# indrajeetadityaroy9/rabitq-ann-search

Measured on AMD Instinct MI355X. Metric: qps (search_batch_device, layer-0 hot path end to end) + fastscan_dist_per_s, higher is better.
Workload: dtype u32 popcount / f32; 1 GPU; SIFT1M-class synthetic (int-valued, clustered; SURVEY 8d C2): 1000000x128 f32 (D=128), 4-bit RaBitQ FastScan + exact-L2 rerank, R=32, k=10, 10000 queries per GPU resident in HBM; n_index=1000000, dim=128, bits=4, k=10, nq_per_gpu=10000, index_builder=cphnsw_mi355x (this repo), batch_sets=2, parallelism=query-sharded x1, index replicated

## Files before the change

include/cphnsw_mi355x.h:

```cpp
#ifndef CPHNSW_MI355X_H
#define CPHNSW_MI355X_H

#include <stddef.h>
#include <stdint.h>

#ifdef __cplusplus
extern "C" {
#endif

typedef struct cph_index cph_index;

typedef enum {
    CPH_OK = 0,
    CPH_INVALID_ARGUMENT = 1,
    CPH_RUNTIME_ERROR = 2,
    CPH_OUT_OF_MEMORY = 3,
    CPH_NOT_IMPLEMENTED = 4
} cph_status;

const char* cph_last_error(void);

int cph_version(void);

int cph_create(uint64_t dim, uint64_t bits, int device, cph_index** out);
// ... 229 lines not shown
int cph_debug_time_facets(cph_index* h, int on);
int cph_debug_last_facets_us(cph_index* h, double* us);
int cph_debug_facet_slab(cph_index* h, uint64_t counters);
int cph_host_facet_values(const int32_t* column, uint64_t n_entries, const uint64_t* lims, uint64_t n, uint64_t* U, int32_t* values);
int cph_host_facet_counts(const int32_t* column, uint64_t n_entries, const uint64_t* lims, uint64_t n, const uint32_t* words,
                          const uint32_t* removed, uint32_t m, uint64_t* counts_out);
int cph_host_facet_top(const int32_t* column, uint64_t n_entries, const uint64_t* lims, uint64_t n, const uint32_t* words,
                       const uint32_t* removed, uint32_t m, uint32_t K, int32_t* values_out, uint64_t* counts_out, uint32_t* found_out);
int cph_facet_hook(int device, const uint32_t* codes, uint64_t n_entries, const uint32_t* lims, uint64_t n, uint32_t U,
                   const uint32_t* words, uint32_t m, int path, uint64_t* counts_out, double* kernel_us);

int cph_search(cph_index* h, const float* query, uint64_t k, int64_t* ids, float* dist,
               uint64_t* m);

int cph_get_vectors(cph_index* h, uint64_t first, uint64_t count, float* out);

int cph_set_batch_sets(cph_index* h, uint32_t n_sets);

int cph_set_search_params(cph_index* h, uint32_t slots, uint64_t beam_capacity);

int cph_last_search_stats(cph_index* h, uint64_t out[12]);
int cph_last_query_expansions(cph_index* index, uint32_t* out, uint64_t n);
int cph_order_queries(cph_index* index, const float* keys, uint64_t n, uint32_t* order);

typedef struct cph_multi cph_multi;
int cph_multi_create(uint64_t dim, uint64_t bits, const int* devices, uint32_t n_dev, cph_multi** out);
int cph_multi_destroy(cph_multi* m);
int cph_multi_load(cph_multi* m, const char* path);
int cph_multi_load_native(cph_multi* m, const char* path);
int cph_multi_save(cph_multi* m, const char* path);
int cph_multi_save_native(cph_multi* m, const char* path);
int cph_multi_build(cph_multi* m, const float* vectors, uint64_t n);
int cph_multi_finalize(cph_multi* m);
int cph_multi_size(cph_multi* m, uint64_t* n);
int cph_multi_is_finalized(cph_multi* m, int* flag);
int cph_multi_search_batch(cph_multi* m, const float* queries, uint64_t n, uint64_t k, int64_t* ids, float* dist);
int cph_multi_search_batch_filtered(cph_multi* m, const float* queries, uint64_t n, uint64_t k,
                                    const cph_filter* const* f, int64_t* ids, float* dist);
int cph_multi_search_batch_exact(cph_multi* m, const float* queries, uint64_t n, uint64_t k,
                                 const cph_filter* const* f, int64_t* ids, float* dist);
int cph_multi_search_batch_filters(cph_multi* m, const float* queries, uint64_t n, uint64_t k, const cph_filter* const* filters,
                                   uint32_t n_filters, const int32_t* filter_of, int exact, int64_t* ids, float* dist);
typedef struct cph_multi_range cph_multi_range;
int cph_multi_range_search_begin(cph_multi* m, const float* queries, uint64_t n, const float* radius_host,
                                 const cph_filter* const* f, int exact, uint64_t max_results, cph_multi_range** out,
                                 uint64_t* total);
// ... 190 lines not shown
```

rabitq-ann-search_amd/cphnsw_mi355x/_lib.py:

```python
import ctypes as C
import importlib.util
import os
import sys

from . import build as _build

OK, INVALID_ARGUMENT, RUNTIME_ERROR, OUT_OF_MEMORY, NOT_IMPLEMENTED = range(5)
IDS_INTERNAL, IDS_INPUT = 0, 1
METRIC_L2, METRIC_COSINE = 0, 1
METRIC_IP = 2

SYMBOLS = {
    "cph_last_error": (C.c_char_p, []),
    "cph_version": (C.c_int, []),
    "cph_create": (C.c_int, [C.c_uint64, C.c_uint64, C.c_int, C.POINTER(C.c_void_p)]),
    "cph_destroy": (C.c_int, [C.c_void_p]),
    "cph_load": (C.c_int, [C.c_void_p, C.c_char_p]),
    "cph_save": (C.c_int, [C.c_void_p, C.c_char_p]),
    "cph_save_native": (C.c_int, [C.c_void_p, C.c_char_p]),
    "cph_load_native": (C.c_int, [C.c_void_p, C.c_char_p]),
    "cph_size": (C.c_int, [C.c_void_p, C.POINTER(C.c_uint64)]),
    "cph_dim": (C.c_int, [C.c_void_p, C.POINTER(C.c_uint64)]),
    "cph_is_finalized": (C.c_int, [C.c_void_p, C.POINTER(C.c_int)]),
    "cph_build": (C.c_int, [C.c_void_p, C.c_void_p, C.c_uint64]),
# ... 183 lines not shown
    "cph_facet_counts": (C.c_int, [C.c_void_p, C.c_int, C.c_uint32, C.c_void_p, C.c_uint32, C.c_void_p]),
    "cph_facet_top": (C.c_int, [C.c_void_p, C.c_int, C.c_uint32, C.c_void_p, C.c_uint32, C.c_uint32, C.c_void_p, C.c_void_p, C.c_void_p]),
    "cph_debug_time_facets": (C.c_int, [C.c_void_p, C.c_int]),
    "cph_debug_last_facets_us": (C.c_int, [C.c_void_p, C.POINTER(C.c_double)]),
    "cph_debug_facet_slab": (C.c_int, [C.c_void_p, C.c_uint64]),
    "cph_host_facet_values": (C.c_int, [C.c_void_p, C.c_uint64, C.c_void_p, C.c_uint64, C.POINTER(C.c_uint64), C.c_void_p]),
    "cph_host_facet_counts": (C.c_int, [C.c_void_p, C.c_uint64, C.c_void_p, C.c_uint64, C.c_void_p, C.c_void_p, C.c_uint32, C.c_void_p]),
    "cph_host_facet_top": (C.c_int, [C.c_void_p, C.c_uint64, C.c_void_p, C.c_uint64, C.c_void_p, C.c_void_p, C.c_uint32, C.c_uint32,
                                     C.c_void_p, C.c_void_p, C.c_void_p]),
    "cph_facet_hook": (C.c_int, [C.c_int, C.c_void_p, C.c_uint64, C.c_void_p, C.c_uint64, C.c_uint32, C.c_void_p, C.c_uint32, C.c_int,
                                 C.c_void_p, C.POINTER(C.c_double)]),
    "cph_multi_set_tags": (C.c_int, [C.c_void_p, C.c_uint32, C.c_void_p, C.c_void_p, C.c_uint64, C.c_int]),
    "cph_parts_set_tags": (C.c_int, [C.c_void_p, C.c_uint32, C.c_void_p, C.c_void_p, C.c_uint64]),
    "cph_parts_filters_from_tags": (C.c_int, [C.c_void_p, C.c_uint32, C.c_void_p, C.c_void_p, C.c_void_p, C.c_uint32, C.c_void_p]),
    "cph_synchronize": (C.c_int, [C.c_void_p]),
    "cph_set_batch_sets": (C.c_int, [C.c_void_p, C.c_uint32]),
    "cph_search": (C.c_int, [C.c_void_p, C.c_void_p, C.c_uint64, C.c_void_p, C.c_void_p,
                             C.POINTER(C.c_uint64)]),
    "cph_get_vectors": (C.c_int, [C.c_void_p, C.c_uint64, C.c_uint64, C.c_void_p]),
    "cph_set_search_params": (C.c_int, [C.c_void_p, C.c_uint32, C.c_uint64]),
    "cph_last_search_stats": (C.c_int, [C.c_void_p, C.POINTER(C.c_uint64)]),
    "cph_last_query_expansions": (C.c_int, [C.c_void_p, C.c_void_p, C.c_uint64]),
    "cph_order_queries": (C.c_int, [C.c_void_p, C.c_void_p, C.c_uint64, C.c_void_p]),
    "cph_multi_create": (C.c_int, [C.c_uint64, C.c_uint64, C.c_void_p, C.c_uint32, C.POINTER(C.c_void_p)]),
    "cph_multi_destroy": (C.c_int, [C.c_void_p]),
    "cph_multi_load": (C.c_int, [C.c_void_p, C.c_char_p]),
    "cph_multi_load_native": (C.c_int, [C.c_void_p, C.c_char_p]),
    "cph_multi_save": (C.c_int, [C.c_void_p, C.c_char_p]),
    "cph_multi_save_native": (C.c_int, [C.c_void_p, C.c_char_p]),
    "cph_multi_build": (C.c_int, [C.c_void_p, C.c_void_p, C.c_uint64]),
    "cph_multi_finalize": (C.c_int, [C.c_void_p]),
    "cph_multi_size": (C.c_int, [C.c_void_p, C.POINTER(C.c_uint64)]),
    "cph_multi_is_finalized": (C.c_int, [C.c_void_p, C.POINTER(C.c_int)]),
    "cph_multi_search_batch": (C.c_int, [C.c_void_p, C.c_void_p, C.c_uint64, C.c_uint64, C.c_void_p, C.c_void_p]),
    "cph_multi_search_batch_filtered": (C.c_int, [C.c_void_p, C.c_void_p, C.c_uint64, C.c_uint64, C.c_void_p,
                                                  C.c_void_p, C.c_void_p]),
    "cph_multi_search": (C.c_int, [C.c_void_p, C.c_void_p, C.c_uint64, C.c_void_p, C.c_void_p,
                                   C.POINTER(C.c_uint64)]),
    "cph_multi_has_row_map": (C.c_int, [C.c_void_p, C.POINTER(C.c_int)]),
    "cph_multi_set_row_map": (C.c_int, [C.c_void_p, C.c_void_p, C.c_uint64]),
    "cph_multi_set_result_ids": (C.c_int, [C.c_void_p, C.c_int]),
    "cph_multi_set_min_shard": (C.c_int, [C.c_void_p, C.c_uint64]),
    "cph_multi_last_search_stats": (C.c_int, [C.c_void_p, C.POINTER(C.c_uint64)]),
    "cph_multi_last_query_expansions": (C.c_int, [C.c_void_p, C.c_void_p, C.c_uint64]),
    "cph_multi_num_replicas": (C.c_int, [C.c_void_p, C.POINTER(C.c_uint32)]),
    "cph_multi_replica": (C.c_int, [C.c_void_p, C.c_uint32, C.POINTER(C.c_void_p)]),
# ... 153 lines not shown
```

rabitq-ann-search_amd/cphnsw_mi355x/index.py:

```python
import ctypes as C

import numpy as np

from . import _lib

DEFAULT_K = 10


def _as_f32(a):
    return np.ascontiguousarray(np.asarray(a), dtype=np.float32)


def pack_allowed_bits(mask):
    m = np.asarray(mask, dtype=bool).ravel()
    nw = (m.size + 31) // 32
    padded = np.zeros(nw * 32, dtype=np.uint64)
    padded[:m.size] = m
    return (padded.reshape(nw, 32) << np.arange(32, dtype=np.uint64)).sum(axis=1).astype(np.uint32)


class IdFilter:

    def __init__(self, index, words, n_bits, count, input_rows=False):
        self._h = C.c_void_p()
# ... 1972 lines not shown
        return dict(zip(keys, [int(x) for x in out]))

    def synchronize(self):
        for h in self._replicas():
            _lib.check(_lib.lib().cph_synchronize(h))

    def last_query_expansions(self, n):
        out = np.empty(int(n), np.uint32)
        if self._p is not None:
            _lib.check(_lib.lib().cph_parts_last_query_expansions(self._p, out.ctypes.data, int(n)))
        elif self._m is not None:
            _lib.check(_lib.lib().cph_multi_last_query_expansions(self._m, out.ctypes.data, int(n)))
        else:
            _lib.check(_lib.lib().cph_last_query_expansions(self._h, out.ctypes.data, int(n)))
        return out

    def order_queries(self, keys):
        self._no_parts("order_queries")
        keys = np.ascontiguousarray(keys, np.float32)
        out = np.empty(len(keys), np.uint32)
        _lib.check(_lib.lib().cph_order_queries(self._h, keys.ctypes.data, len(keys), out.ctypes.data))
        return out

    def get_vectors(self, first=0, count=None, stored=False):
        self._no_parts("get_vectors")
        if count is None:
            count = self.size - first
        out = np.empty((count, self._sdim), np.float32)
        _lib.check(_lib.lib().cph_get_vectors(self._h, int(first), int(count), out.ctypes.data))
        return out if stored or self._sdim == self._dim else np.ascontiguousarray(out[:, :self._dim])

    def internal_to_input_rows(self, base, chunk=1 << 18):
        base = _as_f32(base)
        key = {}
        for i in range(base.shape[0] - 1, -1, -1):
            key[base[i].tobytes()] = i
        out = np.empty(self.size, np.int64)
        for lo in range(0, self.size, chunk):
            v = self.get_vectors(lo, min(chunk, self.size - lo))
            for j in range(v.shape[0]):
                out[lo + j] = key[v[j].tobytes()]
        return out

    def encode_query(self, query):
        self._no_parts("encode_query")
        q = _as_f32(query)
# ... 192 lines not shown
```

rabitq-ann-search_amd/csrc/cphnsw_mi355x.hip:

```cpp
#include <hip/hip_runtime.h>

#include <algorithm>
#include <atomic>
#include <cfloat>
#include <chrono>
#include <condition_variable>
#include <deque>
#include <functional>
#include <memory>
#include <mutex>
#include <new>
#include <shared_mutex>
#include <string>
#include <thread>
#include <vector>

#include "../../include/cphnsw_mi355x.h"
#include "cph_core.h"
#include "device_buf.h"
#include "device_encode.h"
#include "device_fastscan.h"
#include "device_search.h"
#include "device_stream.h"
#include "device_heap_test.h"
// ... 75 lines not shown
#define CPH_LAUNCH(KERNEL, bits, D, grid, block, lds, st, args)                                   \
    do {                                                                                          \
        if ((D) == 128) CPH_LAUNCH_BITS(KERNEL, bits, 128, grid, block, lds, st, args);           \
        else if ((D) == 1024) CPH_LAUNCH_BITS(KERNEL, bits, 1024, grid, block, lds, st, args);    \
        else CPH_LAUNCH_BITS(KERNEL, bits, 0, grid, block, lds, st, args);                        \
        HIP_CHECK(hipGetLastError());                                                             \
    } while (0)

__global__ void scan_counts_kernel(const uint8_t* blocks, uint64_t n, uint32_t stride, uint32_t count_off, uint32_t* flags) {
    const uint64_t v = (uint64_t)blockIdx.x * blockDim.x + threadIdx.x;
    if (v >= n) return;
    const uint32_t cnt = *reinterpret_cast<const uint32_t*>(blocks + v * stride + count_off);
    if (cnt & 7u) atomicOr(flags, 2u);
}

}

struct BatchSet {
    DevBuf<float> d_queries_raw, d_queries, d_entry_dist, d_dist;
    DevBuf<uint4> d_qmasks;
    DevBuf<QueryHeader> d_qhdr;
    DevBuf<int64_t> d_ids;
    DevBuf<uint32_t> d_count, d_status, d_order, d_redo;
    DevBuf<unsigned long long> d_stats;
    unsigned long long* pin_stats = nullptr;
    uint8_t* pin_io = nullptr;
    uint8_t* pin_io_dev = nullptr;
    size_t pin_io_bytes = 0;
    DevBuf<uint32_t> d_bitmaps, d_logids;
    DevBuf<uint32_t> d_beam, d_beam_tail;
    uint32_t slots = 0;
    uint64_t cap = 0;
    DevBuf<uint32_t> r_bitmaps, r_logids;
    DevBuf<uint32_t> r_beam, r_beam_tail;
    uint32_t r_slots = 0;
    hipEvent_t ev0 = nullptr, ev1 = nullptr, ev_done = nullptr;
    bool used = false;
    uint32_t nq = 0;
    uint32_t run_slots = 0;
    uint64_t run_cap = 0;
    DevBuf<float> x_qpad, x_qnorm;
    DevBuf<unsigned long long> x_pools;
    DevBuf<uint32_t> x_counts;
    bool stats_in_hbm = false;
    StagedTable tab;
    DevBuf<uint32_t> d_redo2;
// ... 142 lines not shown
    DevBuf<uint32_t> d_nbr_info;
    UpperLayerDev layers[kMaxUpperLayers];
    int32_t dev_max_level = 0;
    float norm_factor = 0.0f, inv_sqrt_d = 0.0f;
    NativeMapping native_map;
    const uint8_t* own_view = nullptr;
    std::vector<uint8_t> own_store;
    BatchSet sets[kMaxBatchSets + kLeaderSlots];
    int n_sets = 2;
    int last_set = kMaxBatchSets - 1;
    int last_search = -1;
    bool last_range = false;
    uint64_t range_exact = 0;
    std::vector<std::unique_ptr<RangeScratch>> range_scratch;
    RerankScratch rerank_scratch[kMaxBatchSets];
    int last_rerank = kMaxBatchSets - 1;
    struct PassTimer {
        hipEvent_t ev0 = nullptr, ev1 = nullptr;
        bool on = false, timed = false;
    } pass_timer[kPassKinds];
    uint64_t index_epoch = 0;
    hipStream_t own_stream = nullptr;
    bool order_queries = true;
    uint32_t want_slots = 0;
    uint64_t want_cap = 0;
    uint64_t auto_cap = 0;
    bool pf_off = false;
    bool pf_dense = false;
    std::mutex mu;
    SearchCoalescer coal;
    struct LeaderSlot {
        hipStream_t stream = nullptr;
        uint8_t* pin = nullptr;
        uint8_t* pin_dev = nullptr;
        size_t pin_bytes = 0;
        uint32_t seq = 0;
        uint64_t cur_n = 0, cur_k = 0;
    } leaders[kLeaderSlots];

    void use_device() const { HIP_CHECK(hipSetDevice(device)); }
    uint64_t size() const { return host.n + tail; }
};

namespace {

bool probe_first(const cph_index* h) {
// ... 330 lines not shown
    hi.search_data.assign(n * hi.RL.vertex_bytes, 0);
    const size_t chunk = std::max<size_t>(1, std::min<size_t>(n, (512u << 20) / stride));
    std::vector<uint8_t> stage(chunk * stride);
    for (size_t base = 0; base < n; base += chunk) {
        const size_t c = std::min(chunk, n - base);
        download_blocks(h->d_blocks.p + base * stride, c, h->L, stage.data());
        parallel_for(c, 256, [&](size_t lo, size_t hi_) {
            for (size_t v = lo; v < hi_; ++v) {
                uint8_t* dst = &hi.search_data[(base + v) * hi.RL.vertex_bytes];
                if (h->own_view) std::memcpy(dst, h->own_view + (base + v) * own_stride, own_stride);
                repack_dev_to_ref(&stage[v * stride], h->L, hi.RL, dst + hi.RL.nb_off);
            }
        });
    }
}

void init_set(BatchSet& s) {
    if (s.ev0) return;
    HIP_CHECK(hipEventCreate(&s.ev0));
    HIP_CHECK(hipEventCreate(&s.ev1));
    HIP_CHECK(hipEventCreateWithFlags(&s.ev_done, hipEventDisableTiming));
    HIP_CHECK(hipHostMalloc(reinterpret_cast<void**>(&s.pin_stats), kStatWords * 8, hipHostMallocDefault));
    std::memset(s.pin_stats, 0, kStatWords * 8);
}

BatchSet& next_set(cph_index* h, hipStream_t st) {
    h->last_set = (h->last_set + 1) % h->n_sets;
    BatchSet& s = h->sets[h->last_set];
    init_set(s);
    for (BatchSet& o : h->sets) {
        if (!(o.used && o.ev_done && !o.stats_in_hbm && hipEventQuery(o.ev_done) == hipSuccess)) continue;
        const uint64_t reruns = o.pin_stats[kStatReruns], stage2_reruns = stage2_stat(o, kStatStage2Reruns);
        if (reruns > stage2_reruns && o.cap < h->host.n + 1)
            h->auto_cap = std::max<uint64_t>(h->auto_cap, std::min<uint64_t>(h->host.n + 1, o.cap * 4));
        if (stage2_reruns * 50 > o.nq) h->pf_off = true;
        if (o.pin_stats[kStatExpansions] >= 10000) {
            const double new_per_exp = (double)o.pin_stats[kStatNew] / (double)o.pin_stats[kStatExpansions];
            const double off = h->bits == 4 ? 6.0 : 2.8, on = h->bits == 4 ? 4.5 : 2.2;
            if (new_per_exp > off) h->pf_dense = true;
            else if (new_per_exp < on) h->pf_dense = false;
        }
    }
    if (s.used) HIP_CHECK(hipStreamWaitEvent(st, s.ev_done, 0));
    return s;
}

void stage_queries(cph_index* h, BatchSet& s, const float* d_raw_q, uint64_t nq, hipStream_t st) {
    const HostIndex& hi = h->host;
    const uint32_t D = (uint32_t)hi.D, PW = h->L.PW;
    if (hi.entry == kInvalidNode || hi.entry >= hi.n)
        throw std::runtime_error("Search failed: invalid entry point after finalize.");
    if (s.d_queries.n < nq * D || s.d_qmasks.n < nq * PW || s.d_qhdr.n < nq) {
        if (s.used) HIP_CHECK(hipEventSynchronize(s.ev_done));
        s.d_queries.alloc(nq * D);
        s.d_qmasks.alloc(nq * PW);
        s.d_qhdr.alloc(nq);
        s.d_entry_dist.alloc(nq);
        s.d_order.alloc(nq);
    }
    EncodeArgs a{};
    a.queries_raw = d_raw_q;
    a.nq = (uint32_t)nq;
    a.dim = (uint32_t)hi.dim;
    a.D = D;
    a.PW = PW;
    a.signs = h->d_signs.p;
    a.norm_factor = h->norm_factor;
    a.inv_sqrt_d = h->inv_sqrt_d;
    a.raw = h->d_raw.p;
    a.n = hi.n;
    a.entry = hi.entry;
    a.max_level = h->dev_max_level;
    for (int l = 0; l < kMaxUpperLayers; ++l) a.layers[l] = h->layers[l];
    a.queries_padded = s.d_queries.p;
    a.qmasks = s.d_qmasks.p;
    a.qhdr = s.d_qhdr.p;
    a.entry_dist = s.d_entry_dist.p;
    const uint32_t grid = (uint32_t)std::min<uint64_t>(nq, (uint64_t)h->num_cus * 32);
    hipLaunchKernelGGL(encode_kernel, dim3(grid), dim3(64), encode_lds_bytes(D), st, a);
    HIP_CHECK(hipGetLastError());
}

const float* upload_queries(cph_index* h, BatchSet& s, const float* queries, uint64_t nq, hipStream_t st, bool stored = false) {
    const uint64_t width = stored ? h->dim : h->dim_in;
    if (s.d_queries_raw.n < nq * width) {
        if (s.used) HIP_CHECK(hipEventSynchronize(s.ev_done));
        s.d_queries_raw.alloc(nq * width);
    }
    HIP_CHECK(hipMemcpyAsync(s.d_queries_raw.p, queries, nq * width * 4, hipMemcpyHostToDevice, st));
    return s.d_queries_raw.p;
}

const float* metric_queries(cph_index* h, BatchSet& s, const float* d_raw_q, uint64_t nq, hipStream_t st) {
    if (h->metric == CPH_METRIC_L2 || !d_raw_q || nq == 0) return d_raw_q;
    if (s.m_queries.n < nq * h->dim || (h->metric == CPH_METRIC_IP && s.m_c.n < nq)) {
        if (s.used) HIP_CHECK(hipEventSynchronize(s.ev_done));
        s.m_queries.alloc(nq * h->dim);
        if (h->metric == CPH_METRIC_IP) s.m_c.alloc(nq);
    }
    if (h->metric == CPH_METRIC_IP) {
// ... 346 lines not shown
    f.ids = d_ids;
    f.dist = d_dist;
    f.out_count = d_count;
    f.done_flags = done.flags;
    f.done_seq = done.seq;
    for (uint32_t q0 = 0; q0 < nq; q0 += pl.tile_q) {
        a.s.q_first = f.q_first = q0;
        a.s.q_count = f.q_count = std::min(pl.tile_q, nq - q0);
        CPH_LAUNCH_SCAN(tail_scan_kernel, a.s.D, dim3(pl.P, (f.q_count + pl.gq - 1) / pl.gq), (size_t)pl.C * 8 + (size_t)pl.gq * 8, st, a);
        tail_fold(f, st);
    }
}

void enqueue_search(cph_index* h, BatchSet& s, uint32_t nq, uint32_t k, int64_t* d_ids, float* d_dist,
                    hipStream_t st, uint32_t* d_count_out = nullptr, DoneFlags done = DoneFlags(),
                    const cph_filter* filter = nullptr, const float* d_raw_q = nullptr) {
    const uint64_t n = h->host.n;
    if (s.d_count.n < nq) {
        if (s.used) HIP_CHECK(hipEventSynchronize(s.ev_done));
        s.d_count.alloc(nq);
        s.d_status.alloc(nq);
        s.d_redo.alloc(nq);
    }
    s.d_stats.alloc(kStatWords);
    HIP_CHECK(hipMemsetAsync(s.d_stats.p, 0, kStatWords * 8, st));
    if (filter && filter->popcount == 0) {
        uint32_t* d_count = d_count_out ? d_count_out : s.d_count.p;
        HIP_CHECK(hipEventRecord(s.ev0, st));
        HIP_CHECK(hipMemsetAsync(d_ids, 0xFF, (size_t)nq * k * 8, st));
        HIP_CHECK(hipMemsetD32Async(reinterpret_cast<hipDeviceptr_t>(d_dist), (int)0x7F7FFFFF, (size_t)nq * k, st));
        HIP_CHECK(hipMemsetAsync(d_count, 0, (size_t)nq * 4, st));
        HIP_CHECK(hipMemsetAsync(s.d_status.p, 0, (size_t)nq * 4, st));
        s.run_slots = 0;
        s.run_cap = 0;
        s.nq = nq;
        finish_batch(h, s, st);
        return;
    }
    const uint32_t* d_allow = filter ? filter->words.p : nullptr;
    const bool ordered = size_search(h, s, nq, k, st);
    const uint32_t slots = s.run_slots;
    s.nq = nq;
    const uint32_t* d_order = nullptr;
    if (nq > slots && ordered) {
        hipLaunchKernelGGL(order_kernel, dim3(1), dim3(1024), 0, st, s.d_entry_dist.p, nq, s.d_order.p);
        HIP_CHECK(hipGetLastError());
        d_order = s.d_order.p;
    }
    uint32_t* d_count = d_count_out ? d_count_out : s.d_count.p;
    HIP_CHECK(hipEventRecord(s.ev0, st));
    const bool tail = h->tail != 0;
    ExactPlan tail_plan{};
    if (tail) {
        if (!d_raw_q) throw std::runtime_error("a search of an index with added rows needs the raw queries");
        tail_plan = tail_begin(h, s, d_raw_q, nq, k, st);
    }
    const DoneFlags graph_done = tail ? DoneFlags() : done;
    const bool rerun = s.cap < n + 1 || (d_allow == nullptr && probe_first(h));
    if (rerun && nq <= s.r_slots && !h->want_cap && !h->want_slots) {
        s.run_slots = nq;
        s.run_cap = n + 1;
        launch_search(h, s, nq, k, d_ids, d_dist, d_count, nullptr, Launch::Direct, st, graph_done, d_allow);
    } else {
        launch_search(h, s, nq, k, d_ids, d_dist, d_count, d_order, Launch::Main, st, graph_done, d_allow);
        if (rerun) launch_search(h, s, nq, k, d_ids, d_dist, d_count, nullptr, Launch::Rerun, st, graph_done, d_allow);
    }
    if (tail) tail_finish(h, s, tail_plan, nq, k, d_allow, d_ids, d_dist, d_count, done, st);
    finish_batch(h, s, st);
}
// ... 389 lines not shown
            metric_scores(h, s, d_ids, d_dist, n, k, st);
        };
        if (c.on_device) enqueue(c.q, c.ids, c.dist);
        else with_host_io(h, s, c, true, st, enqueue);
        return;
    }
    if (c.F && !c.filters) throw InvalidArg("null argument");
    const cph_filter* f = c.F ? c.filters[0] : nullptr;
    if (!batch_has_work(h, f, c.q, n, k, c.ids, c.dist)) return;
    h->use_device();
    const std::shared_ptr<const cph_filter> eff = effective_filter(h, f);
    f = eff.get();
    const bool exact = takes_exact(h, f, k, c.exact);
    if (!exact) require_tail_k(h, k);
    hipStream_t st = c.on_device ? c.stream : own_stream(h);
    BatchSet& s = next_set(h, st);
    const bool empty = f && f->popcount == 0;
    auto enqueue = [&](const float* d_q, int64_t* d_ids, float* d_dist) {
        if (!empty) d_q = metric_queries(h, s, d_q, n, st);
        if (exact) {
            enqueue_exact(h, s, d_q, (uint32_t)n, (uint32_t)k, f, d_ids, d_dist, st);
            return metric_scores(h, s, d_ids, d_dist, n, k, st);
        }
        if (!empty) stage_queries(h, s, d_q, n, st);
        enqueue_search(h, s, (uint32_t)n, (uint32_t)k, d_ids, d_dist, st, nullptr, DoneFlags(), f, d_q);
        if (!empty) metric_scores(h, s, d_ids, d_dist, n, k, st);
    };
    if (c.on_device) return enqueue(c.q, c.ids, c.dist);
    if (!exact && !empty && n <= kSmallBatch && n * k <= (1u << 20)) {
        const PinnedIo io(n, k, h->dim_in, 0);
        if (s.pin_io_bytes < io.need && s.used) HIP_CHECK(hipEventSynchronize(s.ev_done));
        grow_pinned(s.pin_io, s.pin_io_dev, s.pin_io_bytes, io.need);
        std::memcpy(io.queries(s.pin_io), c.q, n * h->dim_in * sizeof(float));
        const float* d_q = metric_queries(h, s, io.queries(s.pin_io_dev), n, st);
        stage_queries(h, s, d_q, n, st);
        enqueue_search(h, s, (uint32_t)n, (uint32_t)k, io.ids(s.pin_io_dev), io.dist(s.pin_io_dev), st, io.counts(s.pin_io_dev),
                       DoneFlags(), f, d_q);
        metric_scores(h, s, io.ids(s.pin_io_dev), io.dist(s.pin_io_dev), n, k, st);
        HIP_CHECK(hipStreamSynchronize(st));
        std::memcpy(c.ids, io.ids(s.pin_io), n * k * 8);
        std::memcpy(c.dist, io.dist(s.pin_io), n * k * 4);
        return;
    }
    with_host_io(h, s, c, !empty, st, enqueue);
}

void search_batch(cph_index* h, const BatchCall& c) {
// ... 23 lines not shown
    return guarded([&] {
        if (!out) throw InvalidArg("out must not be null");
        *out = nullptr;
        if (bits != 1 && bits != 2 && bits != 4)
            throw InvalidArg("Unsupported bits=" + std::to_string(bits) + ". Supported: 1, 2, 4.");
        const size_t pd = next_pow2(dim);
        if (dim == 0) throw InvalidArg("dim must be > 0");
        if (pd < 16 || pd > 2048)
            throw InvalidArg("Unsupported dimension " + std::to_string(dim) + " (padded to " + std::to_string(pd) +
                             "). Supported padded dims: 16, 32, 64, 128, 256, 512, 1024, 2048.");
        int ndev = 0;
        if (hipGetDeviceCount(&ndev) != hipSuccess || ndev <= 0)
            throw std::runtime_error("No HIP device available: the MI355X path has no CPU fallback.");
        if (device < 0 || device >= ndev) throw InvalidArg("invalid device ordinal");
        auto* h = new cph_index();
        h->dim = dim;
        h->dim_in = dim;
        h->bits = (uint32_t)bits;
        h->D = (uint32_t)pd;
        h->device = device;
        hipDeviceProp_t prop;
        if (hipGetDeviceProperties(&prop, device) == hipSuccess) h->num_cus = prop.multiProcessorCount;
        if (const char* e = getenv("CPH_QUERY_ORDER")) h->order_queries = atoi(e) != 0;
        if (const char* e = getenv("CPH_LEADER_SLOTS")) h->coal.n_slots = std::max(1, std::min(kLeaderSlots, atoi(e)));
        if (const char* e = getenv("CPH_EXACT_SCRATCH_MB")) h->exact_scratch_bytes = (size_t)std::max(1, atoi(e)) << 20;
        if (const char* e = getenv("CPH_GATHER_US")) h->coal.gather_us = std::max(0, atoi(e));
        if (const char* e = getenv("CPH_WAVES_PER_CU")) { h->waves_per_cu = (uint32_t)std::max(1, atoi(e)); h->waves_from_env = true; }
        *out = h;
    });
}

}

static void refuse_borrowed(const cph_index* h, const char* what) {
    if (h->borrowed)
        throw InvalidArg(std::string(what) + " on a replica of a multi-device index: call it on the multi-device handle");
}
static void refuse_host_less(const cph_index* h, const char* what) {
    if (h->host_less)
        throw InvalidArg(std::string(what) + " on a replica that keeps no host arrays: use replica 0");
}

static void destroy_index(cph_index* h) {
    (void)hipSetDevice(h->device);
    for (auto& s : h->sets) {
        if (s.used && s.ev_done) (void)hipEventSynchronize(s.ev_done);
// ... 652 lines not shown
int cph_synchronize(cph_index* h) {
    return guarded([&] {
        if (!h) throw InvalidArg("null handle");
        std::lock_guard<std::mutex> lk(h->mu);
        h->use_device();
        quiesce(h);
    });
}

int cph_order_queries(cph_index* h, const float* keys, uint64_t n, uint32_t* order) {
    return guarded([&] {
        if (!h || !keys || !order) throw InvalidArg("null argument");
        if (n == 0 || n > 0xFFFFFFFFull) throw InvalidArg("bad n");
        std::lock_guard<std::mutex> lk(h->mu);
        h->use_device();
        DevBuf<float> dk;
        DevBuf<uint32_t> dord;
        dk.alloc(n);
        dord.alloc(n);
        HIP_CHECK(hipMemcpy(dk.p, keys, n * 4, hipMemcpyHostToDevice));
        hipLaunchKernelGGL(order_kernel, dim3(1), dim3(1024), 0, nullptr, dk.p, (uint32_t)n, dord.p);
        HIP_CHECK(hipGetLastError());
        HIP_CHECK(hipMemcpy(order, dord.p, n * 4, hipMemcpyDeviceToHost));
    });
}

int cph_search_batch(cph_index* h, const float* queries, uint64_t n, uint64_t k, int64_t* ids,
                     float* dist) {
    return cph_search_batch_filtered(h, queries, n, k, nullptr, ids, dist);
}

int cph_search_batch_device(cph_index* h, const float* d_queries, uint64_t n, uint64_t k,
                            int64_t* d_ids, float* d_dist, void* stream) {
    return cph_search_batch_device_filtered(h, d_queries, n, k, nullptr, d_ids, d_dist, stream);
}

int cph_filter_create(cph_index* h, const uint32_t* words, uint64_t n_bits, cph_filter** out) {
    return guarded([&] {
        if (!h || !out || (!words && n_bits != 0)) throw InvalidArg("null argument");
        *out = nullptr;
        if (n_bits > 0xFFFFFFFFull) throw InvalidArg("filter too large");
        const uint64_t nw = (n_bits + 31) / 32;
        std::vector<uint32_t> w(words, words + nw);
        if (n_bits & 31) w[nw - 1] &= (1u << (n_bits & 31)) - 1u;
        uint64_t pc = 0;
        for (uint32_t x : w) pc += (uint64_t)__builtin_popcount(x);
// ... 5375 lines not shown
```

rabitq-ann-search_amd/csrc/device_encode.h:

```cpp
#pragma once
#include <hip/hip_runtime.h>

#include <cstddef>

#include "cph_core.h"
#include "device_fastscan.h"

namespace cph {

struct UpperLayerDev {
    const uint32_t* nodes;
    const uint32_t* offsets;
    const uint32_t* nbrs;
    const uint32_t* row_of;
    const uint32_t* nbr_info;
    uint32_t n_nodes;
};

constexpr int kMaxUpperLayers = 24;

struct EncodeArgs {
    const float* queries_raw;
    uint32_t nq, dim, D, PW;
    const float* signs;
    float norm_factor, inv_sqrt_d;
    const float* raw;
    uint64_t n;
    uint32_t entry;
    int32_t max_level;
    UpperLayerDev layers[kMaxUpperLayers];
    float* queries_padded;
    uint4* qmasks;
    QueryHeader* qhdr;
    float* entry_dist;
};

__device__ __forceinline__ void wave_fht(float* x, uint32_t D, int lane) {
    for (uint32_t h = 1; h < D; h <<= 1) {
        for (uint32_t b = lane; b < D / 2; b += 64) {
            const uint32_t i = (b / h) * 2 * h + (b % h);
            const float lo = x[i], hi = x[i + h];
            x[i] = lo + hi;
            x[i + h] = (h < 8) ? (hi - lo) : (lo - hi);
        }
        __syncthreads();
    }
}

template <int N, int QR>
__device__ __forceinline__ void pair_l2_part(const float* q_lds, const float* __restrict__ v, float (&c)[4]) {
    float4 r[N], q[QR];
#pragma unroll
    for (int j = 0; j < N; ++j) r[j] = *reinterpret_cast<const float4*>(v + 8 * j);
#pragma unroll
    for (int j = 0; j < QR; ++j) q[j] = *reinterpret_cast<const float4*>(q_lds + 8 * j);
    __builtin_amdgcn_sched_barrier(0);
#pragma unroll
    for (int j = 0; j < N; ++j) {
// ... 35 lines not shown
    pos = bp;
}
__device__ __forceinline__ int fresh_lane(int lane) {
    asm volatile("" : "+v"(lane));
    return lane;
}

__device__ __forceinline__ UpperLayerDev load_layer(int idx) {
    static_assert(sizeof(UpperLayerDev) == 48 && offsetof(UpperLayerDev, n_nodes) == 40, "six qwords per descriptor");
    using kbyte = const __attribute__((address_space(4))) unsigned char;
    using kqword = const __attribute__((address_space(4))) uint64_t;
    kbyte* seg = (kbyte*)__builtin_amdgcn_kernarg_segment_ptr();
    kqword* w = reinterpret_cast<kqword*>(seg + offsetof(EncodeArgs, layers) + (size_t)idx * sizeof(UpperLayerDev));
    UpperLayerDev L;
    L.nodes = reinterpret_cast<const uint32_t*>(w[0]);
    L.offsets = reinterpret_cast<const uint32_t*>(w[1]);
    L.nbrs = reinterpret_cast<const uint32_t*>(w[2]);
    L.row_of = reinterpret_cast<const uint32_t*>(w[3]);
    L.nbr_info = reinterpret_cast<const uint32_t*>(w[4]);
    L.n_nodes = (uint32_t)w[5];
    return L;
}

__host__ __device__ inline size_t encode_lds_bytes(uint32_t D) { return (size_t)D * 8; }

__global__ __launch_bounds__(64) void encode_kernel(EncodeArgs a) {
    extern __shared__ __align__(16) unsigned char smem[];
    float* qv = reinterpret_cast<float*>(smem);
    float* x = qv + a.D;
    const uint32_t D = a.D;
    for (uint32_t qi = blockIdx.x; qi < a.nq; qi += gridDim.x) {
        const int lane = fresh_lane(threadIdx.x);
        for (uint32_t d = lane; d < D; d += 64) {
            float v = d < a.dim ? a.queries_raw[(size_t)qi * a.dim + d] : 0.0f;
            qv[d] = v;
            x[d] = v;
            a.queries_padded[(size_t)qi * D + d] = v;
        }
        __syncthreads();
        for (int l = 0; l < 3; ++l) {
            for (uint32_t d = lane; d < D; d += 64) x[d] = x[d] * a.signs[l * D + d];
            __syncthreads();
            wave_fht(x, D, lane);
        }
        for (uint32_t d = lane; d < D; d += 64) x[d] = x[d] * a.norm_factor;
        __syncthreads();
        float vmin = x[lane < (int)D ? lane : 0], vmx = vmin;
        uint32_t imin = lane < (int)D ? lane : 0, imax = imin;
        for (uint32_t d = lane + 64; d < D; d += 64) {
            const float v = x[d];
            if (v < vmin) { vmin = v; imin = d; }
            if (v > vmx) { vmx = v; imax = d; }
        }
// ... 128 lines not shown
                            const float od = __shfl_xor(cand, o);
                            const uint32_t oi = __shfl_xor(cand_id, o);
                            const uint32_t op = __shfl_xor(cand_pos, o);
                            if (od < cand || (od == cand && op < cand_pos)) { cand = od; cand_id = oi; cand_pos = op; }
                        }
                        cand = uniform_f32(cand);
                        cand_id = uniform_u32(cand_id);
                        if (cand_id != kInvalidNode && cand < best) {
                            best = cand;
                            best_id = cand_id;
                            improved = true;
                        }
                    }
                }
                ep = best_id;
                ep_dist = best;
            }
        }
        hd.entry = ep;
        if (lane == 0) {
            a.qhdr[qi] = hd;
            if (a.entry_dist) a.entry_dist[qi] = ep_dist;
        }
        __syncthreads();
    }
}

constexpr uint32_t kOrderBuckets = 16384;
__global__ __launch_bounds__(1024) void order_kernel(const float* __restrict__ key, uint32_t nq,
                                                     uint32_t* __restrict__ order) {
    __shared__ uint32_t hist[kOrderBuckets];
    __shared__ uint32_t wsum[16];
    const uint32_t tid = threadIdx.x;
    for (uint32_t b = tid; b < kOrderBuckets; b += 1024) hist[b] = 0;
    __syncthreads();
    for (uint32_t i = tid; i < nq; i += 1024) {
        const uint32_t kb = __float_as_uint(key[i]);
        const uint32_t b = (kb & 0x80000000u) ? 0u : (kb >> 17);
        atomicAdd(&hist[b < kOrderBuckets ? b : kOrderBuckets - 1], 1u);
    }
    __syncthreads();
    uint32_t local[16], run = 0;
#pragma unroll
    for (int j = 0; j < 16; ++j) { local[j] = run; run += hist[tid * 16 + j]; }
    uint32_t inc = run;
    for (int o = 1; o < 64; o <<= 1) {
        const uint32_t v = __shfl_up(inc, o);
        if ((tid & 63) >= (uint32_t)o) inc += v;
    }
    if ((tid & 63) == 63) wsum[tid >> 6] = inc;
    __syncthreads();
    uint32_t base = inc - run;
    for (uint32_t w = 0; w < (tid >> 6); ++w) base += wsum[w];
    __syncthreads();
#pragma unroll
    for (int j = 0; j < 16; ++j) hist[tid * 16 + j] = base + local[j];
    __syncthreads();
    for (uint32_t i = tid; i < nq; i += 1024) {
        const uint32_t kb = __float_as_uint(key[i]);
        const uint32_t b = (kb & 0x80000000u) ? 0u : (kb >> 17);
        const uint32_t pos = atomicAdd(&hist[b < kOrderBuckets ? b : kOrderBuckets - 1], 1u);
        order[pos] = i;
    }
}

}
```

Before: 6.911 million queries/s.

## Fuse query ordering and stats zeroing into encode kernel tail

```diff
diff --git a/include/cphnsw_mi355x.h b/include/cphnsw_mi355x.h
--- a/include/cphnsw_mi355x.h
+++ b/include/cphnsw_mi355x.h
@@ -275,6 +275,9 @@
 int cph_last_search_stats(cph_index* h, uint64_t out[12]);
 int cph_last_query_expansions(cph_index* index, uint32_t* out, uint64_t n);
 int cph_order_queries(cph_index* index, const float* keys, uint64_t n, uint32_t* order);
+int cph_debug_stage_order(cph_index* index, const float* queries, uint64_t nq, uint32_t* order_out, float* keys_out,
+                          uint64_t* stats_out);
+int cph_debug_prologue_fused(cph_index* index, int* fused);
 
 typedef struct cph_multi cph_multi;
 int cph_multi_create(uint64_t dim, uint64_t bits, const int* devices, uint32_t n_dev, cph_multi** out);
diff --git a/rabitq-ann-search_amd/cphnsw_mi355x/_lib.py b/rabitq-ann-search_amd/cphnsw_mi355x/_lib.py
--- a/rabitq-ann-search_amd/cphnsw_mi355x/_lib.py
+++ b/rabitq-ann-search_amd/cphnsw_mi355x/_lib.py
@@ -229,6 +229,8 @@
     "cph_last_search_stats": (C.c_int, [C.c_void_p, C.POINTER(C.c_uint64)]),
     "cph_last_query_expansions": (C.c_int, [C.c_void_p, C.c_void_p, C.c_uint64]),
     "cph_order_queries": (C.c_int, [C.c_void_p, C.c_void_p, C.c_uint64, C.c_void_p]),
+    "cph_debug_stage_order": (C.c_int, [C.c_void_p, C.c_void_p, C.c_uint64, C.c_void_p, C.c_void_p, C.c_void_p]),
+    "cph_debug_prologue_fused": (C.c_int, [C.c_void_p, C.POINTER(C.c_int)]),
     "cph_multi_create": (C.c_int, [C.c_uint64, C.c_uint64, C.c_void_p, C.c_uint32, C.POINTER(C.c_void_p)]),
     "cph_multi_destroy": (C.c_int, [C.c_void_p]),
     "cph_multi_load": (C.c_int, [C.c_void_p, C.c_char_p]),
diff --git a/rabitq-ann-search_amd/cphnsw_mi355x/index.py b/rabitq-ann-search_amd/cphnsw_mi355x/index.py
--- a/rabitq-ann-search_amd/cphnsw_mi355x/index.py
+++ b/rabitq-ann-search_amd/cphnsw_mi355x/index.py
@@ -2018,6 +2018,18 @@
         _lib.check(_lib.lib().cph_order_queries(self._h, keys.ctypes.data, len(keys), out.ctypes.data))
         return out
 
+    def debug_stage_order(self, queries):
+        self._no_parts("debug_stage_order")
+        q = _as_f32(queries)
+        nq = q.shape[0]
+        order = np.empty(nq, np.uint32)
+        keys = np.empty(nq, np.float32)
+        stats = np.empty(20, np.uint64)
+        _lib.check(_lib.lib().cph_debug_stage_order(self._h, q.ctypes.data, nq, order.ctypes.data, keys.ctypes.data, stats.ctypes.data))
+        fused = C.c_int(0)
+        _lib.check(_lib.lib().cph_debug_prologue_fused(self._h, C.byref(fused)))
+        return order, keys, stats, bool(fused.value)
+
     def get_vectors(self, first=0, count=None, stored=False):
         self._no_parts("get_vectors")
         if count is None:
diff --git a/rabitq-ann-search_amd/csrc/cphnsw_mi355x.hip b/rabitq-ann-search_amd/csrc/cphnsw_mi355x.hip
--- a/rabitq-ann-search_amd/csrc/cphnsw_mi355x.hip
+++ b/rabitq-ann-search_amd/csrc/cphnsw_mi355x.hip
@@ -121,6 +121,8 @@
     DevBuf<QueryHeader> d_qhdr;
     DevBuf<int64_t> d_ids;
     DevBuf<uint32_t> d_count, d_status, d_order, d_redo;
+    DevBuf<uint32_t> d_order_hist, d_order_rank;
+    bool enc_prologue = false;
     DevBuf<unsigned long long> d_stats;
     unsigned long long* pin_stats = nullptr;
     uint8_t* pin_io = nullptr;
@@ -309,6 +311,9 @@
     uint64_t index_epoch = 0;
     hipStream_t own_stream = nullptr;
     bool order_queries = true;
+    bool prologue = true;
+    uint64_t prologue_max_nq = 32768;
+    bool debug_prologue = false;
     uint32_t want_slots = 0;
     uint64_t want_cap = 0;
     uint64_t auto_cap = 0;
@@ -685,12 +690,14 @@
     HIP_CHECK(hipEventCreateWithFlags(&s.ev_done, hipEventDisableTiming));
     HIP_CHECK(hipHostMalloc(reinterpret_cast<void**>(&s.pin_stats), kStatWords * 8, hipHostMallocDefault));
     std::memset(s.pin_stats, 0, kStatWords * 8);
+    s.d_stats.alloc(kStatWords);
 }
 
 BatchSet& next_set(cph_index* h, hipStream_t st) {
     h->last_set = (h->last_set + 1) % h->n_sets;
     BatchSet& s = h->sets[h->last_set];
     init_set(s);
+    s.enc_prologue = false;
     for (BatchSet& o : h->sets) {
         if (!(o.used && o.ev_done && !o.stats_in_hbm && hipEventQuery(o.ev_done) == hipSuccess)) continue;
         const uint64_t reruns = o.pin_stats[kStatReruns], stage2_reruns = stage2_stat(o, kStatStage2Reruns);
@@ -708,7 +715,7 @@
     return s;
 }
 
-void stage_queries(cph_index* h, BatchSet& s, const float* d_raw_q, uint64_t nq, hipStream_t st) {
+void stage_queries(cph_index* h, BatchSet& s, const float* d_raw_q, uint64_t nq, hipStream_t st, bool for_batch = false) {
     const HostIndex& hi = h->host;
     const uint32_t D = (uint32_t)hi.D, PW = h->L.PW;
     if (hi.entry == kInvalidNode || hi.entry >= hi.n)
@@ -720,6 +727,12 @@
         s.d_qhdr.alloc(nq);
         s.d_entry_dist.alloc(nq);
         s.d_order.alloc(nq);
+        s.d_order_rank.alloc(nq);
+    }
+    s.enc_prologue = for_batch && h->prologue && h->dev_max_level > 0 && h->order_queries && nq > 64 && nq <= h->prologue_max_nq;
+    if (s.enc_prologue && !s.d_order_hist.p) {
+        s.d_order_hist.alloc(kOrderBuckets + 4);
+        HIP_CHECK(hipMemsetAsync(s.d_order_hist.p, 0, (kOrderBuckets + 4) * 4, st));
     }
     EncodeArgs a{};
     a.queries_raw = d_raw_q;
@@ -739,6 +752,13 @@
     a.qmasks = s.d_qmasks.p;
     a.qhdr = s.d_qhdr.p;
     a.entry_dist = s.d_entry_dist.p;
+    if (s.enc_prologue) {
+        a.order_hist = s.d_order_hist.p;
+        a.order_rank = s.d_order_rank.p;
+        a.order = s.d_order.p;
+        a.stats_zero = s.d_stats.p;
+        a.stats_words = kStatWords;
+    }
     const uint32_t grid = (uint32_t)std::min<uint64_t>(nq, (uint64_t)h->num_cus * 32);
     hipLaunchKernelGGL(encode_kernel, dim3(grid), dim3(64), encode_lds_bytes(D), st, a);
     HIP_CHECK(hipGetLastError());
@@ -1131,8 +1151,9 @@
         s.d_status.alloc(nq);
         s.d_redo.alloc(nq);
     }
-    s.d_stats.alloc(kStatWords);
-    HIP_CHECK(hipMemsetAsync(s.d_stats.p, 0, kStatWords * 8, st));
+    const bool prologue = s.enc_prologue;
+    s.enc_prologue = false;
+    if (!prologue) HIP_CHECK(hipMemsetAsync(s.d_stats.p, 0, kStatWords * 8, st));
     if (filter && filter->popcount == 0) {
         uint32_t* d_count = d_count_out ? d_count_out : s.d_count.p;
         HIP_CHECK(hipEventRecord(s.ev0, st));
@@ -1152,8 +1173,10 @@
     s.nq = nq;
     const uint32_t* d_order = nullptr;
     if (nq > slots && ordered) {
-        hipLaunchKernelGGL(order_kernel, dim3(1), dim3(1024), 0, st, s.d_entry_dist.p, nq, s.d_order.p);
-        HIP_CHECK(hipGetLastError());
+        if (!prologue) {
+            hipLaunchKernelGGL(order_kernel, dim3(1), dim3(1024), 0, st, s.d_entry_dist.p, nq, s.d_order.p);
+            HIP_CHECK(hipGetLastError());
+        }
         d_order = s.d_order.p;
     }
     uint32_t* d_count = d_count_out ? d_count_out : s.d_count.p;
@@ -1589,7 +1612,7 @@
             enqueue_exact(h, s, d_q, (uint32_t)n, (uint32_t)k, f, d_ids, d_dist, st);
             return metric_scores(h, s, d_ids, d_dist, n, k, st);
         }
-        if (!empty) stage_queries(h, s, d_q, n, st);
+        if (!empty) stage_queries(h, s, d_q, n, st, true);
         enqueue_search(h, s, (uint32_t)n, (uint32_t)k, d_ids, d_dist, st, nullptr, DoneFlags(), f, d_q);
         if (!empty) metric_scores(h, s, d_ids, d_dist, n, k, st);
     };
@@ -1659,6 +1682,10 @@
         hipDeviceProp_t prop;
         if (hipGetDeviceProperties(&prop, device) == hipSuccess) h->num_cus = prop.multiProcessorCount;
         if (const char* e = getenv("CPH_QUERY_ORDER")) h->order_queries = atoi(e) != 0;
+        if (const char* e = getenv("CPH_PROLOGUE")) {
+            h->prologue = atoi(e) != 0;
+            if (atoi(e) > 1) h->prologue_max_nq = (uint64_t)atoi(e);
+        }
         if (const char* e = getenv("CPH_LEADER_SLOTS")) h->coal.n_slots = std::max(1, std::min(kLeaderSlots, atoi(e)));
         if (const char* e = getenv("CPH_EXACT_SCRATCH_MB")) h->exact_scratch_bytes = (size_t)std::max(1, atoi(e)) << 20;
         if (const char* e = getenv("CPH_GATHER_US")) h->coal.gather_us = std::max(0, atoi(e));
@@ -2357,6 +2384,44 @@
         hipLaunchKernelGGL(order_kernel, dim3(1), dim3(1024), 0, nullptr, dk.p, (uint32_t)n, dord.p);
         HIP_CHECK(hipGetLastError());
         HIP_CHECK(hipMemcpy(order, dord.p, n * 4, hipMemcpyDeviceToHost));
+    });
+}
+
+int cph_debug_stage_order(cph_index* h, const float* queries, uint64_t nq, uint32_t* order_out, float* keys_out, uint64_t* stats_out) {
+    return guarded([&] {
+        if (!h || !queries || !order_out || !keys_out || !stats_out) throw InvalidArg("null argument");
+        if (nq == 0 || nq > 0xFFFFFFull) throw InvalidArg("bad nq");
+        std::lock_guard<std::mutex> lk(h->mu);
+        require_finalized(h);
+        h->use_device();
+        hipStream_t st = own_stream(h);
+        BatchSet& s = next_set(h, st);
+        stage_queries(h, s, upload_queries(h, s, queries, nq, st, true), nq, st, true);
+        h->debug_prologue = s.enc_prologue;
+        const bool ordered = h->dev_max_level > 0 && h->order_queries;
+        if (!s.enc_prologue) {
+            HIP_CHECK(hipMemsetAsync(s.d_stats.p, 0, kStatWords * 8, st));
+            if (ordered) {
+                hipLaunchKernelGGL(order_kernel, dim3(1), dim3(1024), 0, st, s.d_entry_dist.p, (uint32_t)nq, s.d_order.p);
+                HIP_CHECK(hipGetLastError());
+            }
+        }
+        s.enc_prologue = false;
+        HIP_CHECK(hipEventRecord(s.ev_done, st));
+        s.used = true;
+        HIP_CHECK(hipStreamSynchronize(st));
+        if (ordered) HIP_CHECK(hipMemcpy(order_out, s.d_order.p, nq * 4, hipMemcpyDeviceToHost));
+        else for (uint64_t i = 0; i < nq; ++i) order_out[i] = (uint32_t)i;
+        HIP_CHECK(hipMemcpy(keys_out, s.d_entry_dist.p, nq * 4, hipMemcpyDeviceToHost));
+        HIP_CHECK(hipMemcpy(stats_out, s.d_stats.p, kStatWords * 8, hipMemcpyDeviceToHost));
+    });
+}
+
+int cph_debug_prologue_fused(cph_index* h, int* fused) {
+    return guarded([&] {
+        if (!h || !fused) throw InvalidArg("null argument");
+        std::lock_guard<std::mutex> lk(h->mu);
+        *fused = h->debug_prologue ? 1 : 0;
     });
 }
 
diff --git a/rabitq-ann-search_amd/csrc/device_encode.h b/rabitq-ann-search_amd/csrc/device_encode.h
--- a/rabitq-ann-search_amd/csrc/device_encode.h
+++ b/rabitq-ann-search_amd/csrc/device_encode.h
@@ -33,7 +33,19 @@
     uint4* qmasks;
     QueryHeader* qhdr;
     float* entry_dist;
+    uint32_t* order_hist;
+    uint32_t* order_rank;
+    uint32_t* order;
+    unsigned long long* stats_zero;
+    uint32_t stats_words;
 };
+
+constexpr uint32_t kOrderBuckets = 16384;
+__device__ __forceinline__ uint32_t order_bucket(float key) {
+    const uint32_t kb = __float_as_uint(key);
+    const uint32_t b = (kb & 0x80000000u) ? 0u : (kb >> 17);
+    return b < kOrderBuckets ? b : kOrderBuckets - 1;
+}
 
 __device__ __forceinline__ void wave_fht(float* x, uint32_t D, int lane) {
     for (uint32_t h = 1; h < D; h <<= 1) {
@@ -115,6 +127,62 @@
     return L;
 }
 
+__device__ __forceinline__ uint32_t agent_load(const uint32_t* p) {
+    return __hip_atomic_load(p, __ATOMIC_RELAXED, __HIP_MEMORY_SCOPE_AGENT);
+}
+__device__ __forceinline__ void finish_order(const EncodeArgs& a, int lane) {
+    constexpr int kChunks = kOrderBuckets / 256, kAhead = 8, kQueries = 16;
+    uint4* h4 = reinterpret_cast<uint4*>(a.order_hist) + lane;
+    uint32_t carry = 0;
+    unsigned long long held = 0;
+    for (int j0 = 0; j0 < kChunks; j0 += kAhead) {
+        uint4 v[kAhead];
+#pragma unroll
+        for (int u = 0; u < kAhead; ++u) v[u] = h4[(j0 + u) * 64];
+#pragma unroll
+        for (int u = 0; u < kAhead; ++u) {
+            const uint32_t s = (v[u].x + v[u].y) + (v[u].z + v[u].w);
+            if (__ballot(s != 0) == 0) continue;
+            held |= 1ull << (j0 + u);
+            uint32_t inc = s;
+            for (int o = 1; o < 64; o <<= 1) {
+                const uint32_t t = __shfl_up(inc, o);
+                if (lane >= o) inc += t;
+            }
+            uint4 first;
+            first.x = carry + inc - s;
+            first.y = first.x + v[u].x;
+            first.z = first.y + v[u].y;
+            first.w = first.z + v[u].z;
+            h4[(j0 + u) * 64] = first;
+            carry += (uint32_t)__builtin_amdgcn_readlane((int)inc, 63);
+        }
+    }
+    __builtin_amdgcn_fence(__ATOMIC_RELEASE, "agent");
+    __builtin_amdgcn_fence(__ATOMIC_ACQUIRE, "agent");
+    const uint32_t* key = reinterpret_cast<const uint32_t*>(a.entry_dist);
+    for (uint32_t i0 = 0; i0 < a.nq; i0 += 64 * kQueries) {
+        uint32_t place[kQueries], rank[kQueries];
+#pragma unroll
+        for (int u = 0; u < kQueries; ++u) {
+            const uint32_t i = i0 + u * 64 + lane, ic = i < a.nq ? i : a.nq - 1;
+            place[u] = agent_load(key + ic);
+            rank[u] = agent_load(a.order_rank + ic);
+        }
+#pragma unroll
+        for (int u = 0; u < kQueries; ++u) place[u] = agent_load(a.order_hist + order_bucket(__uint_as_float(place[u])));
+#pragma unroll
+        for (int u = 0; u < kQueries; ++u) {
+            const uint32_t i = i0 + u * 64 + lane, at = place[u] + rank[u];
+            if (i < a.nq && at < a.nq) a.order[at] = i;
+        }
+    }
+    for (int j = 0; j < kChunks; ++j)
+        if ((held >> j) & 1) h4[j * 64] = make_uint4(0, 0, 0, 0);
+    if (lane == 0) a.order_hist[kOrderBuckets] = 0;
+    for (uint32_t w = lane; w < a.stats_words; w += 64) a.stats_zero[w] = 0;
+}
+
 __host__ __device__ inline size_t encode_lds_bytes(uint32_t D) { return (size_t)D * 8; }
 
 __global__ __launch_bounds__(64) void encode_kernel(EncodeArgs a) {
@@ -122,6 +190,7 @@
     float* qv = reinterpret_cast<float*>(smem);
     float* x = qv + a.D;
     const uint32_t D = a.D;
+    bool last = false;
     for (uint32_t qi = blockIdx.x; qi < a.nq; qi += gridDim.x) {
         const int lane = fresh_lane(threadIdx.x);
         for (uint32_t d = lane; d < D; d += 64) {
@@ -296,11 +365,22 @@
             a.qhdr[qi] = hd;
             if (a.entry_dist) a.entry_dist[qi] = ep_dist;
         }
+        if (a.order_hist) {
+            uint32_t ticket = 0;
+            if (lane == 0) {
+                a.order_rank[qi] = __hip_atomic_fetch_add(a.order_hist + order_bucket(ep_dist), 1u, __ATOMIC_RELAXED, __HIP_MEMORY_SCOPE_AGENT);
+                ticket = __hip_atomic_fetch_add(a.order_hist + kOrderBuckets, 1u, __ATOMIC_RELEASE, __HIP_MEMORY_SCOPE_AGENT);
+            }
+            last = uniform_u32(ticket) == a.nq - 1;
+        }
         __syncthreads();
     }
-}
-
-constexpr uint32_t kOrderBuckets = 16384;
+    if (last) {
+        __builtin_amdgcn_fence(__ATOMIC_ACQUIRE, "agent");
+        finish_order(a, fresh_lane(threadIdx.x));
+    }
+}
+
 __global__ __launch_bounds__(1024) void order_kernel(const float* __restrict__ key, uint32_t nq,
                                                      uint32_t* __restrict__ order) {
     __shared__ uint32_t hist[kOrderBuckets];
@@ -309,9 +389,7 @@
     for (uint32_t b = tid; b < kOrderBuckets; b += 1024) hist[b] = 0;
     __syncthreads();
     for (uint32_t i = tid; i < nq; i += 1024) {
-        const uint32_t kb = __float_as_uint(key[i]);
-        const uint32_t b = (kb & 0x80000000u) ? 0u : (kb >> 17);
-        atomicAdd(&hist[b < kOrderBuckets ? b : kOrderBuckets - 1], 1u);
+        atomicAdd(&hist[order_bucket(key[i])], 1u);
     }
     __syncthreads();
     uint32_t local[16], run = 0;
@@ -331,9 +409,7 @@
     for (int j = 0; j < 16; ++j) hist[tid * 16 + j] = base + local[j];
     __syncthreads();
     for (uint32_t i = tid; i < nq; i += 1024) {
-        const uint32_t kb = __float_as_uint(key[i]);
-        const uint32_t b = (kb & 0x80000000u) ? 0u : (kb >> 17);
-        const uint32_t pos = atomicAdd(&hist[b < kOrderBuckets ? b : kOrderBuckets - 1], 1u);
+        const uint32_t pos = atomicAdd(&hist[order_bucket(key[i])], 1u);
         order[pos] = i;
     }
 }
```

Measured after the change: 5.901 million queries/s. 14.6% lower.
